# LarsELund/Bayesian-Neural-Nets

Measured on NVIDIA B200. Metric: train_samples_per_sec, higher is better.
Workload: dtype bf16

## Files before the change

### bayesian-neural-nets_b200/csrc/tc_gemm.cu

```cuda
#include <cuda.h>

#include <cstdlib>

#include "common.cuh"
#include "lrt_chain.cuh"
#include "tc_ptx.cuh"

namespace lbbnn {
namespace {

constexpr int BM = 128, BN = 128, BK = 64;
constexpr int UMMA_K = 16;
constexpr int kStages = 3;
constexpr int kTileBytes = BM * BK * 2;
constexpr int kStageBytes = 4 * kTileBytes;
constexpr int kEpiWarps = 8;
constexpr int kTcThreads = 64 + kEpiWarps * 32;
constexpr int kTmemCols = 512;
constexpr int EW = 16;
constexpr int kBiasBytes = 2 * 2 * BN * 4;
constexpr int kEpiScratchBytes = kEpiWarps * 4096;
static_assert(kEpiScratchBytes >= kBiasBytes, "scratch holds the bias terms too");
constexpr int kSmemBytes = kStages * kStageBytes + 1024  + 256  + kEpiScratchBytes;
constexpr int smem_for(int full, int mode) { return mode == LBBNN_TC_EPI_DW_ADAM ? full : full - kEpiScratchBytes + kBiasBytes; }

using namespace tc;

__host__ __device__ constexpr uint32_t make_idesc(int m, int n, int a_mn, int b_mn) {
  return (1u << 4) | (1u << 7) | (1u << 10) | ((uint32_t)(a_mn & 1) << 15) | ((uint32_t)(b_mn & 1) << 16) |
         ((uint32_t)(n >> 3) << 17) | ((uint32_t)(m >> 4) << 24);
}

__device__ __forceinline__ void umma_bf16(uint32_t tmem_d, uint64_t adesc, uint64_t bdesc, uint32_t idesc, uint32_t accumulate) {
  asm volatile(
      "{\n\t"
      ".reg .pred p;\n\t"
      "setp.ne.b32 p, %4, 0;\n\t"
      "tcgen05.mma.cta_group::1.kind::f16 [%0], %1, %2, %3, p;\n\t"
      "}" ::"r"(tmem_d),
      "l"(adesc), "l"(bdesc), "r"(idesc), "r"(accumulate)
      : "memory");
}

constexpr int kMnBoxBytes = 64 * 128;
__device__ __forceinline__ uint64_t umma_desc_mn_sw128(uint32_t smem_addr) {
  uint64_t d = 0;
  d |= (uint64_t)((smem_addr & 0x3FFFF) >> 4);
  d |= (uint64_t)(kMnBoxBytes >> 4) << 16;
  d |= (uint64_t)(1024 >> 4) << 32;
  d |= (uint64_t)1 << 46;
  d |= (uint64_t)2 << 61;
  return d;
}
__device__ __forceinline__ uint64_t umma_desc(uint32_t smem_addr, int mn) {
  return mn ? umma_desc_mn_sw128(smem_addr) : umma_desc_kmajor_sw128(smem_addr);
}

__device__ __forceinline__ uint32_t pack_bf16(float a, float b) {
  __nv_bfloat162 h = __floats2bfloat162_rn(a, b);
  return *reinterpret_cast<uint32_t*>(&h);
}

struct TcEpi {
  int mode;
  int flags;
  float *d1, *d2;
  const float *bias_mu, *bias_rho;
  Noise noise;
  __nv_bfloat16 *o_bf, *o2_bf, *oT_bf, *o2T_bf;
  float *o_f32, *dsf;
  const __nv_bfloat16* x_bf;
  const float* dsf_prev;
  __nv_bfloat16 *de, *ds, *deT, *dsT;
  float* colsum_part;
  float *p_mu, *p_rho, *p_lam;
  float *m_mu, *m_rho, *m_lam, *v_mu, *v_rho, *v_lam;
  const float* coef;
  lbbnn_priors pri;
  int var_mode;
  float klg, beta1, beta2, adam_eps;
  __nv_bfloat16 *next_M, *next_V;
  double* next_kl_part;
  int a_mn, b_mn;
  int l2_prefetch;
};

__device__ __forceinline__ float4 ld4(const float* p) { return *reinterpret_cast<const float4*>(p); }
__device__ __forceinline__ void st4(float* p, float a, float b, float c, float d) { *reinterpret_cast<float4*>(p) = make_float4(a, b, c, d); }

__device__ __forceinline__ void dw_adam_quad(const TcEpi& e, const chain::Consts& cc, const chain::KlC& kc, float& kl_acc, int64_t off,
                                             const float4 dM, const float4 dV) {
  const float4 mu4 = ld4(e.p_mu + off), rho4 = ld4(e.p_rho + off), lam4 = ld4(e.p_lam + off);
  const float4 mm4 = ld4(e.m_mu + off), mr4 = ld4(e.m_rho + off), ml4 = ld4(e.m_lam + off);
  const float4 vm4 = ld4(e.v_mu + off), vr4 = ld4(e.v_rho + off), vl4 = ld4(e.v_lam + off);
  float mu[4] = {mu4.x, mu4.y, mu4.z, mu4.w}, rho[4] = {rho4.x, rho4.y, rho4.z, rho4.w}, lam[4] = {lam4.x, lam4.y, lam4.z, lam4.w};
  float mm[4] = {mm4.x, mm4.y, mm4.z, mm4.w}, mr[4] = {mr4.x, mr4.y, mr4.z, mr4.w}, ml[4] = {ml4.x, ml4.y, ml4.z, ml4.w};
  float vm[4] = {vm4.x, vm4.y, vm4.z, vm4.w}, vr[4] = {vr4.x, vr4.y, vr4.z, vr4.w}, vl[4] = {vl4.x, vl4.y, vl4.z, vl4.w};
  const float d1[4] = {dM.x, dM.y, dM.z, dM.w}, d2[4] = {dV.x, dV.y, dV.z, dV.w};
#pragma unroll
  for (int t = 0; t < 4; ++t) {
    float gm, gr, gl;
    chain::grads(cc, mu[t], rho[t], lam[t], d1[t], d2[t], gm, gr, gl);
    chain::adam(cc, mu[t], mm[t], vm[t], gm);
    chain::adam(cc, rho[t], mr[t], vr[t], gr);
    chain::adam(cc, lam[t], ml[t], vl[t], gl);
  }
  st4(e.p_mu + off, mu[0], mu[1], mu[2], mu[3]); st4(e.p_rho + off, rho[0], rho[1], rho[2], rho[3]);
  st4(e.p_lam + off, lam[0], lam[1], lam[2], lam[3]);
  st4(e.m_mu + off, mm[0], mm[1], mm[2], mm[3]); st4(e.m_rho + off, mr[0], mr[1], mr[2], mr[3]);
  st4(e.m_lam + off, ml[0], ml[1], ml[2], ml[3]);
  st4(e.v_mu + off, vm[0], vm[1], vm[2], vm[3]); st4(e.v_rho + off, vr[0], vr[1], vr[2], vr[3]);
  st4(e.v_lam + off, vl[0], vl[1], vl[2], vl[3]);
  if (e.next_M) {
    float M[4], V[4];
#pragma unroll
    for (int t = 0; t < 4; ++t) {
      float k_;
      chain::next_moments(kc, cc.var_mode, mu[t], rho[t], lam[t], M[t], V[t], k_);
      kl_acc += k_;
    }
    uint2 pm, pv;
    pm.x = pack_bf16(M[0], M[1]); pm.y = pack_bf16(M[2], M[3]);
    pv.x = pack_bf16(V[0], V[1]); pv.y = pack_bf16(V[2], V[3]);
    *reinterpret_cast<uint2*>(e.next_M + off) = pm;
    *reinterpret_cast<uint2*>(e.next_V + off) = pv;
  }
}

__device__ __forceinline__ void dw_adam_tile(const TcEpi& e, const chain::Consts& cc, const chain::KlC& kc, float& kl_acc, int64_t M,
                                             int64_t N, int64_t row0, int64_t col0, uint32_t tbase, float* __restrict__ stg,
                                             int lane) {
#pragma unroll 1
  for (int c = 0; c < 64 / EW; ++c) {
    float v1[EW], v2[EW];
    tmem_ld16(tbase + c * EW, v1);
    tmem_ld16(tbase + 128 + c * EW, v2);
#pragma unroll
    for (int jj = 0; jj < 4; ++jj) {
      st4(stg + lane * 32 + ((jj ^ (lane & 7)) << 2), v1[4 * jj], v1[4 * jj + 1], v1[4 * jj + 2], v1[4 * jj + 3]);
      st4(stg + lane * 32 + (((4 + jj) ^ (lane & 7)) << 2), v2[4 * jj], v2[4 * jj + 1], v2[4 * jj + 2], v2[4 * jj + 3]);
    }
    __syncwarp();
    const int qd = lane & 3;
    const int64_t col = col0 + c * EW + qd * 4;
#pragma unroll
    for (int it = 0; it < 4; ++it) {
      const int rr = it * 8 + (lane >> 2);
      const float4 dM = ld4(stg + rr * 32 + ((qd ^ (rr & 7)) << 2));
      const float4 dV = ld4(stg + rr * 32 + (((4 + qd) ^ (rr & 7)) << 2));
      const int64_t row = row0 + rr;
      if (row < M && col < N) dw_adam_quad(e, cc, kc, kl_acc, row * N + col, dM, dV);
    }
    __syncwarp();
  }
}

__device__ __forceinline__ float warp_transpose_sum32(float (&vals)[32], int lane) {
#pragma unroll
  for (int s = 16; s >= 1; s >>= 1) {
    const bool up = lane & s;
#pragma unroll
    for (int i = 0; i < s; ++i) {
      const float send = up ? vals[i] : vals[i + s];
      const float keep = up ? vals[i + s] : vals[i];
      vals[i] = keep + __shfl_xor_sync(0xffffffffu, send, s);
    }
  }
  return vals[0];
}

template <int MODE>
__device__ __forceinline__ void epilogue_chunk(const TcEpi& e, const Noise& nz, const chain::Consts& cc, int64_t M, int64_t N,
                                               int64_t row, int64_t col0, const float* __restrict__ sbias, int cl,
                                               const float d1[EW], const float d2[EW]) {
  const bool row_ok = row < M;
  if (!row_ok && !(MODE == LBBNN_TC_EPI_DX && e.colsum_part)) return;
  const bool fullc = col0 + EW - 1 < N;
  if constexpr (MODE == LBBNN_TC_EPI_RAW) {
    float* p1 = e.d1 + row * N + col0;
    float* p2 = e.d2 + row * N + col0;
    if (fullc && (N % 4 == 0)) {
#pragma unroll
      for (int j = 0; j < EW; j += 4) {
        *reinterpret_cast<float4*>(p1 + j) = make_float4(d1[j], d1[j + 1], d1[j + 2], d1[j + 3]);
        *reinterpret_cast<float4*>(p2 + j) = make_float4(d2[j], d2[j + 1], d2[j + 2], d2[j + 3]);
      }
    } else {
#pragma unroll
      for (int j = 0; j < EW; ++j)
        if (col0 + j < N) { p1[j] = d1[j]; p2[j] = d2[j]; }
    }
    return;
  }
  float o[EW], o2[EW];
  if constexpr (MODE == LBBNN_TC_EPI_FWD) {
    float ep[EW];
    if (nz.ptr) {
#pragma unroll
      for (int j = 0; j < EW; ++j) ep[j] = (col0 + j < N) ? __ldg(nz.ptr + row * N + col0 + j) : 0.f;
    } else if (N % 4 == 0) {
#pragma unroll
      for (int j = 0; j < EW; j += 4) philox_normal4(nz.seed, nz.stream, ((uint64_t)row * (uint64_t)N + (uint64_t)(col0 + j)) >> 2, ep + j);
    } else {
#pragma unroll
      for (int j = 0; j < EW; ++j) ep[j] = philox_normal1(nz.seed, nz.stream, (uint64_t)row * (uint64_t)N + (uint64_t)(col0 + j));
    }
#pragma unroll
    for (int j = 0; j < EW; ++j) {
      const int64_t n = col0 + j;
      float v = 0.f, f = 0.f;
      if (n < N) {
        const float sd = sqrtf(fmaxf(d2[j], 0.f) + sbias[BN + cl + j]);
        v = d1[j] + sbias[cl + j] + sd * ep[j];
        f = ep[j] / (2.0f * sd);
        if (e.flags & LBBNN_FLAG_RELU) v = fmaxf(v, 0.f);
      }
      o[j] = v;
      o2[j] = f;
    }
    const bool v4 = fullc && (N % 4 == 0);
    if (e.o_f32 || e.dsf) {
      if (v4) {
#pragma unroll
        for (int j = 0; j < EW; j += 4) {
          if (e.o_f32) *reinterpret_cast<float4*>(e.o_f32 + row * N + col0 + j) = make_float4(o[j], o[j + 1], o[j + 2], o[j + 3]);
          if (e.dsf) *reinterpret_cast<float4*>(e.dsf + row * N + col0 + j) = make_float4(o2[j], o2[j + 1], o2[j + 2], o2[j + 3]);
        }
      } else {
#pragma unroll
        for (int j = 0; j < EW; ++j)
          if (col0 + j < N) {
            if (e.o_f32) e.o_f32[row * N + col0 + j] = o[j];
            if (e.dsf) e.dsf[row * N + col0 + j] = o2[j];
          }
      }
    }
    if (fullc && (N % 8 == 0)) {
#pragma unroll
      for (int j = 0; j < EW; j += 8) {
        uint4 a, b;
        a.x = pack_bf16(o[j], o[j + 1]); a.y = pack_bf16(o[j + 2], o[j + 3]); a.z = pack_bf16(o[j + 4], o[j + 5]); a.w = pack_bf16(o[j + 6], o[j + 7]);
        b.x = pack_bf16(o[j] * o[j], o[j + 1] * o[j + 1]); b.y = pack_bf16(o[j + 2] * o[j + 2], o[j + 3] * o[j + 3]);
        b.z = pack_bf16(o[j + 4] * o[j + 4], o[j + 5] * o[j + 5]); b.w = pack_bf16(o[j + 6] * o[j + 6], o[j + 7] * o[j + 7]);
        if (e.o_bf) *reinterpret_cast<uint4*>(e.o_bf + row * N + col0 + j) = a;
        if (e.o2_bf) *reinterpret_cast<uint4*>(e.o2_bf + row * N + col0 + j) = b;
      }
    } else {
#pragma unroll
      for (int j = 0; j < EW; ++j)
        if (col0 + j < N) {
          if (e.o_bf) e.o_bf[row * N + col0 + j] = __float2bfloat16_rn(o[j]);
          if (e.o2_bf) e.o2_bf[row * N + col0 + j] = __float2bfloat16_rn(o[j] * o[j]);
        }
    }
    if (e.oT_bf) {
#pragma unroll
      for (int j = 0; j < EW; ++j)
        if (col0 + j < N) {
          e.oT_bf[(col0 + j) * M + row] = __float2bfloat16_rn(o[j]);
          e.o2T_bf[(col0 + j) * M + row] = __float2bfloat16_rn(o[j] * o[j]);
        }
    }
    return;
  }
  if constexpr (MODE == LBBNN_TC_EPI_DX) {
  float xv[EW], fv[EW];
  if (!row_ok) {
#pragma unroll
    for (int j = 0; j < EW; ++j) { xv[j] = 0.f; fv[j] = 0.f; }
  } else if (fullc && (N % 8 == 0)) {
#pragma unroll
    for (int j = 0; j < EW; j += 8) {
      const uint4 u = *reinterpret_cast<const uint4*>(e.x_bf + row * N + col0 + j);
      const __nv_bfloat162* h = reinterpret_cast<const __nv_bfloat162*>(&u);
#pragma unroll
      for (int t = 0; t < 4; ++t) {
        const float2 f2 = __bfloat1622float2(h[t]);
        xv[j + 2 * t] = f2.x; xv[j + 2 * t + 1] = f2.y;
      }
    }
#pragma unroll
    for (int j = 0; j < EW; j += 4) {
      const float4 f4 = e.dsf_prev ? *reinterpret_cast<const float4*>(e.dsf_prev + row * N + col0 + j) : make_float4(0.f, 0.f, 0.f, 0.f);
      fv[j] = f4.x; fv[j + 1] = f4.y; fv[j + 2] = f4.z; fv[j + 3] = f4.w;
    }
  } else {
#pragma unroll
    for (int j = 0; j < EW; ++j) {
      const bool ok = col0 + j < N;
      xv[j] = ok ? __bfloat162float(e.x_bf[row * N + col0 + j]) : 0.f;
      fv[j] = (ok && e.dsf_prev) ? e.dsf_prev[row * N + col0 + j] : 0.f;
    }
  }
#pragma unroll
  for (int j = 0; j < EW; ++j) {
    float g = fmaf(2.0f * xv[j], d2[j], d1[j]);
    if ((e.flags & LBBNN_FLAG_MASK_DX) && !(xv[j] > 0.f)) g = 0.f;
    if (!row_ok || col0 + j >= N) g = 0.f;
    o[j] = g;
    o2[j] = g * fv[j];
  }
  if (e.colsum_part) {
    float vals[32];
#pragma unroll
    for (int j = 0; j < EW; ++j) { vals[j] = o[j]; vals[EW + j] = o2[j]; }
// ... 116 lines not shown
      constexpr uint64_t kbs = BMN ? (uint64_t)(2048 >> 4) : (uint64_t)((UMMA_K * 2) >> 4);
      for (int t = blockIdx.x; t < num_tiles; t += gridDim.x, ++it) {
        const int as = it & 1;
        mbar_wait(&tempty_bar[as], ((it >> 1) & 1) ^ 1);
        tc_fence_after();
        const uint32_t d1 = tmem_base + as * 256, d2 = d1 + 128;
        for (int kb = 0; kb < num_kb; ++kb) {
          mbar_wait(&full_bar[stage], phase);
          tc_fence_after();
          const uint32_t sa = smem_u32(smem + stage * kStageBytes);
          const uint64_t a1 = umma_desc(sa + 0 * kTileBytes, AMN), a2 = umma_desc(sa + 1 * kTileBytes, AMN);
          const uint64_t b1 = umma_desc(sa + 2 * kTileBytes, BMN), b2 = umma_desc(sa + 3 * kTileBytes, BMN);
#pragma unroll
          for (int k = 0; k < BK / UMMA_K; ++k) {
            const uint32_t acc = (kb | k) ? 1u : 0u;
            umma_bf16(d1, a1 + k * ka, b1 + k * kbs, idesc, acc);
            umma_bf16(d2, a2 + k * ka, b2 + k * kbs, idesc, acc);
          }
          umma_commit(&empty_bar[stage]);
          if (++stage == kStages) { stage = 0; phase ^= 1; }
        }
        umma_commit(&tfull_bar[as]);
      }
    }
  } else {
    Noise nz = epi.noise;
    nz.resolve();
    chain::Consts cc = {};
    chain::KlC kc = {};
    float kl_acc = 0.f;
    if constexpr (MODE == LBBNN_TC_EPI_DW_ADAM) {
      cc = chain::make_consts(epi.pri, epi.var_mode, epi.klg, epi.beta1, epi.beta2, epi.adam_eps, epi.coef);
      kc = chain::make_klc(epi.pri);
    }
    const int q = warp & 3, half = (warp - 2) >> 2;
    const int et = threadIdx.x - 64;
    int it = 0;
    for (int t = blockIdx.x; t < num_tiles; t += gridDim.x, ++it) {
      const int as = it & 1;
      int mb, nb;
      tile_coords(t, num_m, num_n, mb, nb);
      const int m0 = mb * BM, n0 = nb * BN;
      float* sbias = sbias_all + as * 2 * BN;
      if constexpr (MODE == LBBNN_TC_EPI_FWD) {
        const int c = et & (BN - 1);
        const int64_t n = n0 + c;
        float v = 0.f;
        if (n < N) {
          if (et < BN) v = __ldg(epi.bias_mu + n);
          else { const float sb = sigma_of(__ldg(epi.bias_rho + n)); v = sb * sb; }
        }
        sbias[(et < BN ? 0 : BN) + c] = v;
        asm volatile("bar.sync 1, %0;" ::"n"(kEpiWarps * 32) : "memory");
      }
      mbar_wait(&tfull_bar[as], (it >> 1) & 1);
      tc_fence_after();
      const int64_t row = m0 + q * 32 + lane;
      const uint32_t tbase = tmem_base + ((uint32_t)(q * 32) << 16) + as * 256 + half * 64;
      if constexpr (MODE == LBBNN_TC_EPI_DW_ADAM) {
        dw_adam_tile(epi, cc, kc, kl_acc, M, N, m0 + q * 32, n0 + half * 64, tbase, sbias_all + (warp - 2) * 1024, lane);
      } else {
#pragma unroll 1
        for (int c = 0; c < 64 / EW; ++c) {
          float v1[EW], v2[EW];
          tmem_ld16(tbase + c * EW, v1);
          tmem_ld16(tbase + 128 + c * EW, v2);
          const int cl = half * 64 + c * EW;
          epilogue_chunk<MODE>(epi, nz, cc, M, N, row, n0 + cl, sbias, cl, v1, v2);
        }
      }
      tc_fence_before();
      __syncwarp();
      if (lane == 0) mbar_arrive(&tempty_bar[as]);
    }
    if constexpr (MODE == LBBNN_TC_EPI_DW_ADAM) {
      if (epi.next_kl_part) {
        const float w = warp_sum(kl_acc);
        if (lane == 0) epi.next_kl_part[(int64_t)blockIdx.x * kEpiWarps + (warp - 2)] = (double)w;
      }
    }
  }
  tc_fence_before();
  __syncthreads();
  if (warp == 1) {
    tc_fence_after();
    tmem_dealloc(tmem_base, kTmemCols);
  }
}

constexpr int kStages2 = 4;
constexpr int kBHalfBytes = (BN / 2) * BK * 2;
constexpr int kStageBytes2 = 2 * kTileBytes + 2 * kBHalfBytes;
constexpr int kSmemBytes2 = kStages2 * kStageBytes2 + 1024 + 256 + kEpiScratchBytes;
static_assert(kSmemBytes <= 232448 && kSmemBytes2 <= 232448, "over the 227 KB shared-memory limit");
constexpr int kGroupM2 = kGroupM / 2;
constexpr int kL2Prefetch = 0;

__device__ __forceinline__ void umma_bf16_pair(uint32_t tmem_d, uint64_t adesc, uint64_t bdesc, uint32_t idesc, uint32_t accumulate) {
  asm volatile(
      "{\n\t"
      ".reg .pred p;\n\t"
      "setp.ne.b32 p, %4, 0;\n\t"
      "tcgen05.mma.cta_group::2.kind::f16 [%0], %1, %2, %3, p;\n\t"
      "}" ::"r"(tmem_d),
      "l"(adesc), "l"(bdesc), "r"(idesc), "r"(accumulate)
      : "memory");
}

__device__ __forceinline__ void tile_coords2(int t, int num_m2, int num_n, int group, int& mb2, int& nb) {
  const int per_group = group * num_n;
  const int g = t / per_group, r = t - g * per_group;
  const int m_first = g * group;
  const int gm = min(group, num_m2 - m_first);
  nb = r / gm;
  mb2 = m_first + (r - nb * gm);
}

template <int MODE, int AMN, int BMN>
__global__ void __cluster_dims__(2, 1, 1) __launch_bounds__(kTcThreads, 1)
tc_dual_gemm_bf16_pair(const __grid_constant__ CUtensorMap tmA1, const __grid_constant__ CUtensorMap tmA2,
                       const __grid_constant__ CUtensorMap tmB1, const __grid_constant__ CUtensorMap tmB2, const TcEpi epi,
                       int M, int N, int K, int group) {
  extern __shared__ uint8_t smem_raw[];
  uint8_t* smem = reinterpret_cast<uint8_t*>((reinterpret_cast<uintptr_t>(smem_raw) + 1023) & ~uintptr_t(1023));
  uint64_t* bars = reinterpret_cast<uint64_t*>(smem + kStages2 * kStageBytes2);
  uint64_t* full_bar = bars;
  uint64_t* empty_bar = bars + kStages2;
  uint64_t* tfull_bar = bars + 2 * kStages2;
  uint64_t* tempty_bar = bars + 2 * kStages2 + 2;
  uint32_t* tmem_holder = reinterpret_cast<uint32_t*>(bars + 2 * kStages2 + 4);
  float* sbias_all = reinterpret_cast<float*>(smem + kStages2 * kStageBytes2 + 256);

  const int warp = threadIdx.x >> 5, lane = threadIdx.x & 31;
  const uint32_t rank = cluster_ctarank();
  const int num_m2 = (M + 2 * BM - 1) / (2 * BM), num_n = (N + BN - 1) / BN;
  const int num_tiles = num_m2 * num_n, num_kb = (K + BK - 1) / BK;
  const int cluster_id = blockIdx.x >> 1, num_clusters = gridDim.x >> 1;

  if (warp == 0 && lane == 0) {
    tma_prefetch_desc(&tmA1); tma_prefetch_desc(&tmA2); tma_prefetch_desc(&tmB1); tma_prefetch_desc(&tmB2);
    for (int s = 0; s < kStages2; ++s) { mbar_init(&full_bar[s], 2); mbar_init(&empty_bar[s], 1); }
    for (int s = 0; s < 2; ++s) { mbar_init(&tfull_bar[s], 1); mbar_init(&tempty_bar[s], 2 * kEpiWarps); }
    fence_barrier_init();
  }
  __syncwarp();
  if (warp == 1) tmem_alloc_pair(tmem_holder, kTmemCols);
  tc_fence_before();
  cluster_sync_all();
  tc_fence_after();
  const uint32_t tmem_base = *tmem_holder;

  if (warp == 0) {
    if (lane == 0) {
      int stage = 0; uint32_t phase = 0;
      for (int t = cluster_id; t < num_tiles; t += num_clusters) {
        int mb2, nb;
        tile_coords2(t, num_m2, num_n, group, mb2, nb);
        const int m0 = mb2 * 2 * BM + (int)rank * BM, n0h = nb * BN + (int)rank * (BN / 2);
        for (int kb = 0; kb < num_kb; ++kb) {
          if (epi.l2_prefetch > 0) {
            int pk = kb + epi.l2_prefetch, pm0 = m0, pn0 = n0h;
            bool ok = true;
            if (pk >= num_kb) {
              pk -= num_kb;
              const int tn = t + num_clusters;
              ok = tn < num_tiles && pk < num_kb;
              if (ok) {
                int pmb2, pnb;
                tile_coords2(tn, num_m2, num_n, group, pmb2, pnb);
                pm0 = pmb2 * 2 * BM + (int)rank * BM; pn0 = pnb * BN + (int)rank * (BN / 2);
              }
            }
            if (ok) {
              if constexpr (!AMN) { tma_prefetch_l2_2d(&tmA1, pk * BK, pm0); tma_prefetch_l2_2d(&tmA2, pk * BK, pm0); }
              else {
#pragma unroll
                for (int h = 0; h < 2; ++h) { tma_prefetch_l2_2d(&tmA1, pm0 + 64 * h, pk * BK); tma_prefetch_l2_2d(&tmA2, pm0 + 64 * h, pk * BK); }
              }
              if constexpr (!BMN) { tma_prefetch_l2_2d(&tmB1, pk * BK, pn0); tma_prefetch_l2_2d(&tmB2, pk * BK, pn0); }
              else { tma_prefetch_l2_2d(&tmB1, pn0, pk * BK); tma_prefetch_l2_2d(&tmB2, pn0, pk * BK); }
            }
          }
          mbar_wait(&empty_bar[stage], phase ^ 1);
          uint8_t* sa = smem + stage * kStageBytes2;
          const uint32_t lead_full = mapa_u32(&full_bar[stage], 0);
          mbar_expect_tx_cluster(lead_full, kStageBytes2);
          if constexpr (!AMN) {
            tma_load_2d_pair(sa, &tmA1, lead_full, kb * BK, m0);
            tma_load_2d_pair(sa + kTileBytes, &tmA2, lead_full, kb * BK, m0);
          } else {
#pragma unroll
            for (int h = 0; h < 2; ++h) {
              tma_load_2d_pair(sa + h * kMnBoxBytes, &tmA1, lead_full, m0 + 64 * h, kb * BK);
              tma_load_2d_pair(sa + kTileBytes + h * kMnBoxBytes, &tmA2, lead_full, m0 + 64 * h, kb * BK);
            }
          }
          if constexpr (!BMN) {
            tma_load_2d_pair(sa + 2 * kTileBytes, &tmB1, lead_full, kb * BK, n0h);
            tma_load_2d_pair(sa + 2 * kTileBytes + kBHalfBytes, &tmB2, lead_full, kb * BK, n0h);
          } else {
            tma_load_2d_pair(sa + 2 * kTileBytes, &tmB1, lead_full, n0h, kb * BK);
            tma_load_2d_pair(sa + 2 * kTileBytes + kBHalfBytes, &tmB2, lead_full, n0h, kb * BK);
          }
          if (++stage == kStages2) { stage = 0; phase ^= 1; }
        }
      }
    }
  } else if (warp == 1) {
    if (lane == 0 && rank == 0) {
      int stage = 0; uint32_t phase = 0; int it = 0;
      constexpr uint32_t idesc = make_idesc(2 * BM, BN, AMN, BMN);
      constexpr uint64_t ka = AMN ? (uint64_t)(2048 >> 4) : (uint64_t)((UMMA_K * 2) >> 4);
      constexpr uint64_t kbs = BMN ? (uint64_t)(2048 >> 4) : (uint64_t)((UMMA_K * 2) >> 4);
      for (int t = cluster_id; t < num_tiles; t += num_clusters, ++it) {
        const int as = it & 1;
        mbar_wait(&tempty_bar[as], ((it >> 1) & 1) ^ 1);
        tc_fence_after();
        const uint32_t d1 = tmem_base + as * 256, d2 = d1 + 128;
        for (int kb = 0; kb < num_kb; ++kb) {
          mbar_wait(&full_bar[stage], phase);
          tc_fence_after();
          const uint32_t sa = smem_u32(smem + stage * kStageBytes2);
          const uint64_t a1 = umma_desc(sa, AMN), a2 = umma_desc(sa + kTileBytes, AMN);
          const uint64_t b1 = umma_desc(sa + 2 * kTileBytes, BMN);
          const uint64_t b2 = umma_desc(sa + 2 * kTileBytes + kBHalfBytes, BMN);
#pragma unroll
          for (int k = 0; k < BK / UMMA_K; ++k) {
            const uint32_t acc = (kb | k) ? 1u : 0u;
            umma_bf16_pair(d1, a1 + k * ka, b1 + k * kbs, idesc, acc);
            umma_bf16_pair(d2, a2 + k * ka, b2 + k * kbs, idesc, acc);
          }
          umma_commit_pair(&empty_bar[stage], 3);
          if (++stage == kStages2) { stage = 0; phase ^= 1; }
        }
        umma_commit_pair(&tfull_bar[as], 3);
      }
    }
  } else {
    Noise nz = epi.noise;
    nz.resolve();
    chain::Consts cc = {};
    chain::KlC kc = {};
    float kl_acc = 0.f;
    if constexpr (MODE == LBBNN_TC_EPI_DW_ADAM) {
      cc = chain::make_consts(epi.pri, epi.var_mode, epi.klg, epi.beta1, epi.beta2, epi.adam_eps, epi.coef);
      kc = chain::make_klc(epi.pri);
    }
    const int q = warp & 3, half = (warp - 2) >> 2;
    const int et = threadIdx.x - 64;
    int it = 0;
    for (int t = cluster_id; t < num_tiles; t += num_clusters, ++it) {
      const int as = it & 1;
      int mb2, nb;
      tile_coords2(t, num_m2, num_n, group, mb2, nb);
      const int m0 = mb2 * 2 * BM + (int)rank * BM, n0 = nb * BN;
      float* sbias = sbias_all + as * 2 * BN;
      if constexpr (MODE == LBBNN_TC_EPI_FWD) {
        const int c = et & (BN - 1);
        const int64_t n = n0 + c;
        float v = 0.f;
        if (n < N) {
          if (et < BN) v = __ldg(epi.bias_mu + n);
          else { const float sb = sigma_of(__ldg(epi.bias_rho + n)); v = sb * sb; }
        }
        sbias[(et < BN ? 0 : BN) + c] = v;
        asm volatile("bar.sync 1, %0;" ::"n"(kEpiWarps * 32) : "memory");
      }
      mbar_wait(&tfull_bar[as], (it >> 1) & 1);
      tc_fence_after();
      const int64_t row = m0 + q * 32 + lane;
      const uint32_t tbase = tmem_base + ((uint32_t)(q * 32) << 16) + as * 256 + half * 64;
      if constexpr (MODE == LBBNN_TC_EPI_DW_ADAM) {
        dw_adam_tile(epi, cc, kc, kl_acc, M, N, m0 + q * 32, n0 + half * 64, tbase, sbias_all + (warp - 2) * 1024, lane);
      } else {
#pragma unroll 1
        for (int c = 0; c < 64 / EW; ++c) {
          float v1[EW], v2[EW];
          tmem_ld16(tbase + c * EW, v1);
          tmem_ld16(tbase + 128 + c * EW, v2);
          const int cl = half * 64 + c * EW;
          epilogue_chunk<MODE>(epi, nz, cc, M, N, row, n0 + cl, sbias, cl, v1, v2);
        }
      }
      tc_fence_before();
      __syncwarp();
      if (lane == 0) mbar_arrive_cluster(mapa_u32(&tempty_bar[as], 0));
    }
    if constexpr (MODE == LBBNN_TC_EPI_DW_ADAM) {
      if (epi.next_kl_part) {
        const float w = warp_sum(kl_acc);
        if (lane == 0) epi.next_kl_part[(int64_t)blockIdx.x * kEpiWarps + (warp - 2)] = (double)w;
      }
    }
  }
  __syncwarp();
  tc_fence_before();
  cluster_sync_all();
  if (warp == 1) {
    tc_fence_after();
    tmem_dealloc_pair(tmem_base, kTmemCols);
  }
}

typedef CUresult (*EncodeTiledFn)(CUtensorMap*, CUtensorMapDataType, cuuint32_t, void*, const cuuint64_t*, const cuuint64_t*,
                                  const cuuint32_t*, const cuuint32_t*, CUtensorMapInterleave, CUtensorMapSwizzle,
                                  CUtensorMapL2promotion, CUtensorMapFloatOOBfill);

EncodeTiledFn get_encode() {
  static EncodeTiledFn fn = nullptr;
  if (fn) return fn;
  void* p = nullptr;
  cudaDriverEntryPointQueryResult qres;
  if (cudaGetDriverEntryPoint("cuTensorMapEncodeTiled", &p, cudaEnableDefault, &qres) != cudaSuccess ||
      qres != cudaDriverEntryPointSuccess)
    return nullptr;
  fn = (EncodeTiledFn)p;
  return fn;
}

int make_map(CUtensorMap* map, const void* ptr, int64_t rows, int64_t K, int box_rows = BM) {
  EncodeTiledFn enc = get_encode();
  LBBNN_REQUIRE(enc != nullptr, "cuTensorMapEncodeTiled not available from the driver");
  LBBNN_REQUIRE((reinterpret_cast<uintptr_t>(ptr) & 15) == 0 && (K * 2) % 16 == 0,
                "TMA operand must be 16B aligned with a 16B-multiple row pitch (K %% 8 == 0), K=%lld", (long long)K);
  cuuint64_t dims[2] = {(cuuint64_t)K, (cuuint64_t)rows};
  cuuint64_t strides[1] = {(cuuint64_t)K * 2};
  cuuint32_t box[2] = {(cuuint32_t)BK, (cuuint32_t)box_rows};
  cuuint32_t estr[2] = {1, 1};
  CUresult r = enc(map, CU_TENSOR_MAP_DATA_TYPE_BFLOAT16, 2, const_cast<void*>(ptr), dims, strides, box, estr,
                   CU_TENSOR_MAP_INTERLEAVE_NONE, CU_TENSOR_MAP_SWIZZLE_128B, CU_TENSOR_MAP_L2_PROMOTION_L2_256B,
                   CU_TENSOR_MAP_FLOAT_OOB_FILL_NONE);
  LBBNN_REQUIRE(r == CUDA_SUCCESS, "cuTensorMapEncodeTiled failed (%d) rows=%lld K=%lld", (int)r, (long long)rows, (long long)K);
  return LBBNN_OK;
}

int make_map_mn(CUtensorMap* map, const void* ptr, int64_t rows, int64_t K) {
  EncodeTiledFn enc = get_encode();
  LBBNN_REQUIRE(enc != nullptr, "cuTensorMapEncodeTiled not available from the driver");
  LBBNN_REQUIRE((reinterpret_cast<uintptr_t>(ptr) & 15) == 0 && (rows * 2) % 16 == 0,
                "MN-major TMA operand must be 16B aligned with a 16B-multiple row pitch (rows %% 8 == 0), rows=%lld", (long long)rows);
  cuuint64_t dims[2] = {(cuuint64_t)rows, (cuuint64_t)K};
  cuuint64_t strides[1] = {(cuuint64_t)rows * 2};
  cuuint32_t box[2] = {64u, (cuuint32_t)BK};
  cuuint32_t estr[2] = {1, 1};
  CUresult r = enc(map, CU_TENSOR_MAP_DATA_TYPE_BFLOAT16, 2, const_cast<void*>(ptr), dims, strides, box, estr,
                   CU_TENSOR_MAP_INTERLEAVE_NONE, CU_TENSOR_MAP_SWIZZLE_128B, CU_TENSOR_MAP_L2_PROMOTION_L2_256B,
                   CU_TENSOR_MAP_FLOAT_OOB_FILL_NONE);
  LBBNN_REQUIRE(r == CUDA_SUCCESS, "cuTensorMapEncodeTiled (MN-major) failed (%d) rows=%lld K=%lld", (int)r, (long long)rows, (long long)K);
  return LBBNN_OK;
}

int launch_tc(const void* A1, const void* A2, const void* B1, const void* B2, int64_t M, int64_t N, int64_t K, const TcEpi& epi_in,
              cudaStream_t st) {
  LBBNN_REQUIRE(A1 && A2 && B1 && B2 && M > 0 && N > 0 && K > 0, "bad GEMM operands");
  TcEpi epi = epi_in;
  {
    const char* pf = getenv("LBBNN_TC_L2_PREFETCH");
    epi.l2_prefetch = pf ? atoi(pf) : kL2Prefetch;
  }
  LBBNN_REQUIRE(M < (1LL << 31) && N < (1LL << 31) && K < (1LL << 31), "GEMM dims must fit int32");
  CUtensorMap mA1, mA2, mB1, mB2;
  if (epi.a_mn) {
    if (int rc = make_map_mn(&mA1, A1, M, K)) return rc;
    if (int rc = make_map_mn(&mA2, A2, M, K)) return rc;
  } else {
    if (int rc = make_map(&mA1, A1, M, K)) return rc;
    if (int rc = make_map(&mA2, A2, M, K)) return rc;
  }
  const char* pe = getenv("LBBNN_TC_PAIR");
  const int pair_mode = pe ? atoi(pe) : 1;
  const int64_t tiles2 = ceil_div(M, 2 * BM) * ceil_div(N, BN);
  if (pair_mode && M > BM && (pair_mode == 2 || tiles2 >= sm_count() / 2)) {
    if (epi.b_mn) {
      if (int rc = make_map_mn(&mB1, B1, N, K)) return rc;
      if (int rc = make_map_mn(&mB2, B2, N, K)) return rc;
    } else {
      if (int rc = make_map(&mB1, B1, N, K, BN / 2)) return rc;
      if (int rc = make_map(&mB2, B2, N, K, BN / 2)) return rc;
    }
    const int clusters = (int)(tiles2 < sm_count() / 2 ? tiles2 : sm_count() / 2);
    const char* ge = getenv("LBBNN_TC_GROUP");
    const int group = ge && atoi(ge) > 0 ? atoi(ge) : kGroupM2;
    const int key = epi.mode * 4 + epi.a_mn * 2 + epi.b_mn;
    switch (key) {
#define LBBNN_PAIR_CASE(MODE_, A_, B_)                                                                                                \
  case (MODE_) * 4 + (A_) * 2 + (B_): {                                                                                              \
    static bool attr_set_ = false;                                                                                                   \
    if (!attr_set_) {                                                                                                                \
      LBBNN_CUDA(cudaFuncSetAttribute(tc_dual_gemm_bf16_pair<MODE_, A_, B_>, cudaFuncAttributeMaxDynamicSharedMemorySize,           \
                                      smem_for(kSmemBytes2, MODE_)));                                                               \
      attr_set_ = true;                                                                                                              \
    }                                                                                                                                \
    tc_dual_gemm_bf16_pair<MODE_, A_, B_><<<2 * clusters, kTcThreads, smem_for(kSmemBytes2, MODE_), st>>>(mA1, mA2, mB1, mB2, epi, \
                                                                                                           (int)M, (int)N, (int)K, \
                                                                                                           group);                 \
    break;                                                                                                                           \
  }
      LBBNN_PAIR_CASE(LBBNN_TC_EPI_RAW, 0, 0)
      LBBNN_PAIR_CASE(LBBNN_TC_EPI_RAW, 0, 1)
      LBBNN_PAIR_CASE(LBBNN_TC_EPI_RAW, 1, 0)
      LBBNN_PAIR_CASE(LBBNN_TC_EPI_RAW, 1, 1)
      LBBNN_PAIR_CASE(LBBNN_TC_EPI_FWD, 0, 0)
      LBBNN_PAIR_CASE(LBBNN_TC_EPI_DX, 0, 0)
      LBBNN_PAIR_CASE(LBBNN_TC_EPI_DX, 0, 1)
      LBBNN_PAIR_CASE(LBBNN_TC_EPI_DW_ADAM, 1, 1)
#undef LBBNN_PAIR_CASE
      default: LBBNN_REQUIRE(false, "no kernel for epilogue mode %d with operand majors (%d, %d)", epi.mode, epi.a_mn, epi.b_mn);
    }
    return check_launch("tc_dual_gemm_bf16_pair");
  }
  if (epi.b_mn) {
    if (int rc = make_map_mn(&mB1, B1, N, K)) return rc;
    if (int rc = make_map_mn(&mB2, B2, N, K)) return rc;
  } else {
    if (int rc = make_map(&mB1, B1, N, K)) return rc;
    if (int rc = make_map(&mB2, B2, N, K)) return rc;
  }
  const int64_t tiles = ceil_div(M, BM) * ceil_div(N, BN);
  const int grid = (int)(tiles < sm_count() ? tiles : sm_count());
  const int key = epi.mode * 4 + epi.a_mn * 2 + epi.b_mn;
  switch (key) {
#define LBBNN_ONE_CASE(MODE_, A_, B_)                                                                                          \
  case (MODE_) * 4 + (A_) * 2 + (B_): {                                                                                       \
    static bool attr_set_ = false;                                                                                             \
    if (!attr_set_) {                                                                                                          \
      LBBNN_CUDA(cudaFuncSetAttribute(tc_dual_gemm_bf16<MODE_, A_, B_>, cudaFuncAttributeMaxDynamicSharedMemorySize,          \
                                      smem_for(kSmemBytes, MODE_)));                                                          \
      attr_set_ = true;                                                                                                        \
    }                                                                                                                          \
    tc_dual_gemm_bf16<MODE_, A_, B_><<<grid, kTcThreads, smem_for(kSmemBytes, MODE_), st>>>(mA1, mA2, mB1, mB2, epi, (int)M,   \
                                                                                             (int)N, (int)K);                   \
    break;                                                                                                                     \
  }
    LBBNN_ONE_CASE(LBBNN_TC_EPI_RAW, 0, 0)
    LBBNN_ONE_CASE(LBBNN_TC_EPI_RAW, 0, 1)
    LBBNN_ONE_CASE(LBBNN_TC_EPI_RAW, 1, 0)
    LBBNN_ONE_CASE(LBBNN_TC_EPI_RAW, 1, 1)
    LBBNN_ONE_CASE(LBBNN_TC_EPI_FWD, 0, 0)
    LBBNN_ONE_CASE(LBBNN_TC_EPI_DX, 0, 0)
    LBBNN_ONE_CASE(LBBNN_TC_EPI_DX, 0, 1)
    LBBNN_ONE_CASE(LBBNN_TC_EPI_DW_ADAM, 1, 1)
#undef LBBNN_ONE_CASE
    default: LBBNN_REQUIRE(false, "no kernel for epilogue mode %d with operand majors (%d, %d)", epi.mode, epi.a_mn, epi.b_mn);
  }
  return check_launch("tc_dual_gemm_bf16");
}

}
}

using namespace lbbnn;

extern "C" int lbbnn_tc_dual_gemm_raw(const void* A1, const void* A2, const void* B1, const void* B2, int64_t M, int64_t N,
                                      int64_t K, float* D1, float* D2, lbbnn_stream s) {
  LBBNN_REQUIRE(D1 && D2, "NULL output");
  TcEpi e = {};
  e.mode = LBBNN_TC_EPI_RAW;
  e.d1 = D1; e.d2 = D2;
  return launch_tc(A1, A2, B1, B2, M, N, K, e, (cudaStream_t)s);
}

extern "C" int lbbnn_tc_lrt_fwd(const void* x_bf, const void* x2_bf, const void* M_bf, const void* V_bf, int64_t batch,
                                int64_t in_features, int64_t out_features, const float* bias_mu, const float* bias_rho,
                                const lbbnn_noise* nz, int flags, void* act_bf, void* act2_bf, void* actT_bf, void* act2T_bf,
                                float* ds_factor, float* act_f32, lbbnn_stream s) {
  LBBNN_REQUIRE(bias_mu && bias_rho, "NULL bias");
  LBBNN_REQUIRE((actT_bf == nullptr) == (act2T_bf == nullptr), "transposed outputs come in pairs");
  TcEpi e = {};
  e.mode = LBBNN_TC_EPI_FWD; e.flags = flags;
  e.bias_mu = bias_mu; e.bias_rho = bias_rho; e.noise = make_noise(nz);
  e.o_bf = (__nv_bfloat16*)act_bf; e.o2_bf = (__nv_bfloat16*)act2_bf; e.oT_bf = (__nv_bfloat16*)actT_bf;
  e.o2T_bf = (__nv_bfloat16*)act2T_bf; e.dsf = ds_factor; e.o_f32 = act_f32;
  return launch_tc(x_bf, x2_bf, M_bf, V_bf, batch, out_features, in_features, e, (cudaStream_t)s);
}

extern "C" int lbbnn_tc_lrt_bwd_input(const void* dE_bf, const void* dS_bf, const void* MT_bf, const void* VT_bf, int64_t batch,
                                      int64_t in_features, int64_t out_features, const void* x_bf, const float* ds_factor_prev,
                                      int flags, void* dE_prev_bf, void* dS_prev_bf, void* dE_prevT_bf, void* dS_prevT_bf,
                                      lbbnn_stream s) {
  LBBNN_REQUIRE(x_bf && dE_prev_bf && dS_prev_bf, "NULL argument");
  LBBNN_REQUIRE((dE_prevT_bf == nullptr) == (dS_prevT_bf == nullptr), "transposed outputs come in pairs");
  TcEpi e = {};
  e.mode = LBBNN_TC_EPI_DX; e.flags = flags;
  e.x_bf = (const __nv_bfloat16*)x_bf; e.dsf_prev = ds_factor_prev;
  e.de = (__nv_bfloat16*)dE_prev_bf; e.ds = (__nv_bfloat16*)dS_prev_bf; e.deT = (__nv_bfloat16*)dE_prevT_bf;
  e.dsT = (__nv_bfloat16*)dS_prevT_bf;
  return launch_tc(dE_bf, dS_bf, MT_bf, VT_bf, batch, in_features, out_features, e, (cudaStream_t)s);
}

namespace lbbnn {
namespace {
__global__ void __launch_bounds__(256) colsum_part_reduce(const float* __restrict__ part, int n_part, int64_t cols2,
                                                          float* __restrict__ out) {
  const int64_t c = (int64_t)blockIdx.x * blockDim.x + threadIdx.x;
  if (c >= cols2) return;
  float s = 0.f;
  for (int r = 0; r < n_part; ++r) s += part[(int64_t)r * cols2 + c];
  out[c] = s;
}
}
}

extern "C" int lbbnn_tc_dual_gemm_raw_ex(const void* A1, const void* A2, const void* B1, const void* B2, int64_t M, int64_t N,
                                         int64_t K, int a_mn, int b_mn, float* D1, float* D2, lbbnn_stream s) {
  LBBNN_REQUIRE(D1 && D2, "NULL output");
  TcEpi e = {};
  e.mode = LBBNN_TC_EPI_RAW;
  e.d1 = D1; e.d2 = D2;
  e.a_mn = a_mn ? 1 : 0; e.b_mn = b_mn ? 1 : 0;
  return launch_tc(A1, A2, B1, B2, M, N, K, e, (cudaStream_t)s);
}

extern "C" size_t lbbnn_tc_colsum_part_floats(int64_t batch, int64_t in_features) {
  return (size_t)(ceil_div(batch, 32) * 2 * in_features);
}

extern "C" int lbbnn_tc_colsum_reduce(const float* part, int64_t batch, int64_t in_features, float* colsum, lbbnn_stream s) {
  LBBNN_REQUIRE(part && colsum && batch > 0 && in_features > 0, "bad argument");
  const int64_t cols2 = 2 * in_features;
  colsum_part_reduce<<<(unsigned)ceil_div(cols2, 256), 256, 0, (cudaStream_t)s>>>(part, (int)ceil_div(batch, 32), cols2, colsum);
  return check_launch("colsum_part_reduce");
}

extern "C" int lbbnn_tc_lrt_bwd_input_mn(const void* dE_bf, const void* dS_bf, const void* M_bf, const void* V_bf, int64_t batch,
                                         int64_t in_features, int64_t out_features, const void* x_bf, const float* ds_factor_prev,
                                         int flags, void* dE_prev_bf, void* dS_prev_bf, float* colsum_part, lbbnn_stream s) {
  LBBNN_REQUIRE(x_bf && dE_prev_bf && dS_prev_bf, "NULL argument");
  TcEpi e = {};
  e.mode = LBBNN_TC_EPI_DX; e.flags = flags;
  e.x_bf = (const __nv_bfloat16*)x_bf; e.dsf_prev = ds_factor_prev;
  e.de = (__nv_bfloat16*)dE_prev_bf; e.ds = (__nv_bfloat16*)dS_prev_bf;
  e.colsum_part = colsum_part;
  e.a_mn = 0; e.b_mn = 1;
  return launch_tc(dE_bf, dS_bf, M_bf, V_bf, batch, in_features, out_features, e, (cudaStream_t)s);
}

extern "C" size_t lbbnn_tc_lrt_dw_adam_kl_parts(void) { return (size_t)sm_count() * kEpiWarps; }

extern "C" int lbbnn_tc_lrt_dw_adam_next(const void* dE_bf, const void* dS_bf, const void* x_bf, const void* x2_bf,
                                         const lbbnn_layer* L, int64_t batch, const lbbnn_priors* pri, int var_mode,
                                         float kl_grad, const lbbnn_adam_layer_state* adam, void* next_M_bf, void* next_V_bf,
                                         double* next_kl_part, lbbnn_stream s);

extern "C" int lbbnn_tc_lrt_dw_adam(const void* dE_bf, const void* dS_bf, const void* x_bf, const void* x2_bf,
                                    const lbbnn_layer* L, int64_t batch, const lbbnn_priors* pri, int var_mode,
                                    float kl_grad, const lbbnn_adam_layer_state* adam, lbbnn_stream s) {
  return lbbnn_tc_lrt_dw_adam_next(dE_bf, dS_bf, x_bf, x2_bf, L, batch, pri, var_mode, kl_grad, adam, nullptr, nullptr, nullptr, s);
}

extern "C" int lbbnn_tc_lrt_dw_adam_next(const void* dE_bf, const void* dS_bf, const void* x_bf, const void* x2_bf,
                                         const lbbnn_layer* L, int64_t batch, const lbbnn_priors* pri, int var_mode,
                                         float kl_grad, const lbbnn_adam_layer_state* adam, void* next_M_bf, void* next_V_bf,
                                         double* next_kl_part, lbbnn_stream s) {
  LBBNN_REQUIRE((next_M_bf == nullptr) == (next_V_bf == nullptr), "next_M / next_V come in pairs");
  LBBNN_REQUIRE(next_kl_part == nullptr || next_M_bf != nullptr, "next_kl_part needs next_M / next_V");
  LBBNN_REQUIRE(L && pri && adam && adam->coef, "NULL argument");
  LBBNN_REQUIRE(L->weight_mu && L->weight_rho && L->lambdal && L->in_features > 0 && L->out_features > 0, "bad layer");
  LBBNN_REQUIRE(L->z == nullptr && L->z_kl == nullptr, "the fused update is for LRT layers (no multiplicative z)");
  LBBNN_REQUIRE(L->in_features % 8 == 0 && L->out_features % 8 == 0, "fused dW update needs in/out features divisible by 8");
  for (int i = 0; i < 3; ++i) LBBNN_REQUIRE(adam->exp_avg[i] && adam->exp_avg_sq[i], "NULL Adam state %d", i);
  TcEpi e = {};
  e.mode = LBBNN_TC_EPI_DW_ADAM;
  e.p_mu = const_cast<float*>(L->weight_mu); e.p_rho = const_cast<float*>(L->weight_rho); e.p_lam = const_cast<float*>(L->lambdal);
  e.m_mu = adam->exp_avg[0]; e.m_rho = adam->exp_avg[1]; e.m_lam = adam->exp_avg[2];
  e.v_mu = adam->exp_avg_sq[0]; e.v_rho = adam->exp_avg_sq[1]; e.v_lam = adam->exp_avg_sq[2];
  const float* ptrs[9] = {e.p_mu, e.p_rho, e.p_lam, e.m_mu, e.m_rho, e.m_lam, e.v_mu, e.v_rho, e.v_lam};
  for (int i = 0; i < 9; ++i) LBBNN_REQUIRE((reinterpret_cast<uintptr_t>(ptrs[i]) & 15) == 0, "parameters / Adam state must be 16B aligned");
  e.coef = adam->coef; e.pri = *pri; e.var_mode = var_mode; e.klg = kl_grad;
  e.beta1 = adam->beta1; e.beta2 = adam->beta2; e.adam_eps = adam->eps;
  e.next_M = (__nv_bfloat16*)next_M_bf; e.next_V = (__nv_bfloat16*)next_V_bf; e.next_kl_part = next_kl_part;
  if (next_kl_part)
    LBBNN_CUDA(cudaMemsetAsync(next_kl_part, 0, lbbnn_tc_lrt_dw_adam_kl_parts() * sizeof(double), (cudaStream_t)s));
  e.a_mn = 1; e.b_mn = 1;
  return launch_tc(dE_bf, dS_bf, x_bf, x2_bf, L->out_features, L->in_features, batch, e, (cudaStream_t)s);
}
```

Before: 2.507 million.

## Add staged 256x256 pair GEMM kernel stashing pass results in L2

Adds a new 2-CTA cluster kernel for forward and dX modes. It computes the two GEMMs (mu and variance passes) back to back, each into its own 256-column TMEM accumulator over a 256x256 cluster tile, so each operand tile covers more output per load. Because TMEM cannot hold both full results for the epilogue, the first pass's results are spilled to a per-SM global stash with L2 evict_last hints and read back with evict_first before the fused epilogue. This trades less operand traffic and deeper 6-stage pipelining against extra stash traffic through L2, a one-time host-synchronising allocation, and an assumption of one CTA per SM that is only enforced by the shared-memory size.

```diff
diff --git a/bayesian-neural-nets_b200/csrc/tc_gemm.cu b/bayesian-neural-nets_b200/csrc/tc_gemm.cu
--- a/bayesian-neural-nets_b200/csrc/tc_gemm.cu
+++ b/bayesian-neural-nets_b200/csrc/tc_gemm.cu
@@ -1,6 +1,7 @@
 #include <cuda.h>
 
 #include <cstdlib>
+#include <mutex>
 
 #include "common.cuh"
 #include "lrt_chain.cuh"
@@ -723,6 +724,194 @@
   }
 }
 
+constexpr int kStagesS = 6;
+constexpr int kStageBytesS = 2 * kTileBytes;
+constexpr int kBiasBytesS = 2 * 2 * 2 * BN * 4;
+constexpr int kSmemBytesS = kStagesS * kStageBytesS + 1024 + 256 + kBiasBytesS;
+static_assert(kSmemBytesS <= 232448, "over the 227 KB shared-memory limit");
+static_assert(kSmemBytesS > 232448 / 2, "the stash slot per %smid needs at most one CTA per SM");
+constexpr int kStashFloats = 2 * BM * 2 * BN;
+
+__device__ __forceinline__ uint32_t smid_u32() {
+  uint32_t r;
+  asm volatile("mov.u32 %0, %%smid;" : "=r"(r));
+  return r;
+}
+__device__ __forceinline__ void st_stash(float* p, float a, float b, float c, float d, uint64_t pol) {
+  asm volatile("st.global.L1::no_allocate.L2::cache_hint.v4.f32 [%0], {%1, %2, %3, %4}, %5;" ::"l"(p), "f"(a), "f"(b), "f"(c),
+               "f"(d), "l"(pol)
+               : "memory");
+}
+__device__ __forceinline__ float4 ld_stash(const float* p, uint64_t pol) {
+  float4 v;
+  asm volatile("ld.global.L1::no_allocate.L2::cache_hint.v4.f32 {%0, %1, %2, %3}, [%4], %5;"
+               : "=f"(v.x), "=f"(v.y), "=f"(v.z), "=f"(v.w)
+               : "l"(p), "l"(pol));
+  return v;
+}
+
+template <int MODE, int AMN, int BMN>
+__global__ void __cluster_dims__(2, 1, 1) __launch_bounds__(kTcThreads, 1)
+tc_gemm_bf16_pair_staged(const __grid_constant__ CUtensorMap tmA1, const __grid_constant__ CUtensorMap tmA2,
+                         const __grid_constant__ CUtensorMap tmB1, const __grid_constant__ CUtensorMap tmB2, const TcEpi epi,
+                         int M, int N, int K, int group, float* __restrict__ stash) {
+  extern __shared__ uint8_t smem_raw[];
+  uint8_t* smem = reinterpret_cast<uint8_t*>((reinterpret_cast<uintptr_t>(smem_raw) + 1023) & ~uintptr_t(1023));
+  uint64_t* bars = reinterpret_cast<uint64_t*>(smem + kStagesS * kStageBytesS);
+  uint64_t* full_bar = bars;
+  uint64_t* empty_bar = bars + kStagesS;
+  uint64_t* tfull_bar = bars + 2 * kStagesS;
+  uint64_t* tempty_bar = bars + 2 * kStagesS + 2;
+  uint32_t* tmem_holder = reinterpret_cast<uint32_t*>(bars + 2 * kStagesS + 4);
+  float* sbias_all = reinterpret_cast<float*>(smem + kStagesS * kStageBytesS + 256);
+
+  const int warp = threadIdx.x >> 5, lane = threadIdx.x & 31;
+  const uint32_t rank = cluster_ctarank();
+  const int num_m2 = (M + 2 * BM - 1) / (2 * BM), num_n2 = (N + 2 * BN - 1) / (2 * BN);
+  const int num_tiles = num_m2 * num_n2, num_kb = (K + BK - 1) / BK;
+  const int cluster_id = blockIdx.x >> 1, num_clusters = gridDim.x >> 1;
+
+  if (warp == 0 && lane == 0) {
+    tma_prefetch_desc(&tmA1); tma_prefetch_desc(&tmA2); tma_prefetch_desc(&tmB1); tma_prefetch_desc(&tmB2);
+    for (int s = 0; s < kStagesS; ++s) { mbar_init(&full_bar[s], 2); mbar_init(&empty_bar[s], 1); }
+    for (int s = 0; s < 2; ++s) { mbar_init(&tfull_bar[s], 1); mbar_init(&tempty_bar[s], 2 * kEpiWarps); }
+    fence_barrier_init();
+  }
+  __syncwarp();
+  if (warp == 1) tmem_alloc_pair(tmem_holder, kTmemCols);
+  tc_fence_before();
+  cluster_sync_all();
+  tc_fence_after();
+  const uint32_t tmem_base = *tmem_holder;
+
+  if (warp == 0) {
+    if (lane == 0) {
+      int stage = 0; uint32_t phase = 0;
+      for (int t = cluster_id; t < num_tiles; t += num_clusters) {
+        int mb2, nb2;
+        tile_coords2(t, num_m2, num_n2, group, mb2, nb2);
+        const int m0 = mb2 * 2 * BM + (int)rank * BM, n0h = nb2 * 2 * BN + (int)rank * BN;
+        for (int pass = 0; pass < 2; ++pass) {
+          const CUtensorMap* ta = pass ? &tmA2 : &tmA1;
+          const CUtensorMap* tb = pass ? &tmB2 : &tmB1;
+          for (int kb = 0; kb < num_kb; ++kb) {
+            mbar_wait(&empty_bar[stage], phase ^ 1);
+            uint8_t* sa = smem + stage * kStageBytesS;
+            const uint32_t lead_full = mapa_u32(&full_bar[stage], 0);
+            mbar_expect_tx_cluster(lead_full, kStageBytesS);
+            if constexpr (!AMN) {
+              tma_load_2d_pair(sa, ta, lead_full, kb * BK, m0);
+            } else {
+#pragma unroll
+              for (int h = 0; h < 2; ++h) tma_load_2d_pair(sa + h * kMnBoxBytes, ta, lead_full, m0 + 64 * h, kb * BK);
+            }
+            if constexpr (!BMN) {
+              tma_load_2d_pair(sa + kTileBytes, tb, lead_full, kb * BK, n0h);
+            } else {
+#pragma unroll
+              for (int h = 0; h < 2; ++h) tma_load_2d_pair(sa + kTileBytes + h * kMnBoxBytes, tb, lead_full, n0h + 64 * h, kb * BK);
+            }
+            if (++stage == kStagesS) { stage = 0; phase ^= 1; }
+          }
+        }
+      }
+    }
+  } else if (warp == 1) {
+    if (lane == 0 && rank == 0) {
+      int stage = 0; uint32_t phase = 0; int it = 0;
+      constexpr uint32_t idesc = make_idesc(2 * BM, 2 * BN, AMN, BMN);
+      constexpr uint64_t ka = AMN ? (uint64_t)(2048 >> 4) : (uint64_t)((UMMA_K * 2) >> 4);
+      constexpr uint64_t kbs = BMN ? (uint64_t)(2048 >> 4) : (uint64_t)((UMMA_K * 2) >> 4);
+      for (int t = cluster_id; t < num_tiles; t += num_clusters, ++it) {
+        for (int pass = 0; pass < 2; ++pass) {
+          mbar_wait(&tempty_bar[pass], (it & 1) ^ 1);
+          tc_fence_after();
+          const uint32_t d = tmem_base + pass * 256;
+          for (int kb = 0; kb < num_kb; ++kb) {
+            mbar_wait(&full_bar[stage], phase);
+            tc_fence_after();
+            const uint32_t sa = smem_u32(smem + stage * kStageBytesS);
+            const uint64_t a = umma_desc(sa, AMN), b = umma_desc(sa + kTileBytes, BMN);
+#pragma unroll
+            for (int k = 0; k < BK / UMMA_K; ++k) umma_bf16_pair(d, a + k * ka, b + k * kbs, idesc, (kb | k) ? 1u : 0u);
+            umma_commit_pair(&empty_bar[stage], 3);
+            if (++stage == kStagesS) { stage = 0; phase ^= 1; }
+          }
+          umma_commit_pair(&tfull_bar[pass], 3);
+        }
+      }
+    }
+  } else {
+    Noise nz = epi.noise;
+    nz.resolve();
+    const chain::Consts cc = {};
+    const int q = warp & 3, half = (warp - 2) >> 2;
+    const int et = threadIdx.x - 64;
+    float* slot = stash + (size_t)smid_u32() * kStashFloats + (size_t)(warp - 2) * (2 * 8 * 4 * 32 * 4) + lane * 4;
+    constexpr int kProd = 8 * 4 * 32 * 4;
+    uint64_t pol_keep, pol_drop;
+    asm volatile("createpolicy.fractional.L2::evict_last.b64 %0, 1.0;" : "=l"(pol_keep));
+    asm volatile("createpolicy.fractional.L2::evict_first.b64 %0, 1.0;" : "=l"(pol_drop));
+    int it = 0;
+    for (int t = cluster_id; t < num_tiles; t += num_clusters, ++it) {
+      int mb2, nb2;
+      tile_coords2(t, num_m2, num_n2, group, mb2, nb2);
+      const int m0 = mb2 * 2 * BM + (int)rank * BM, n0 = nb2 * 2 * BN;
+      float* sbias = sbias_all + (it & 1) * 4 * BN;
+      if constexpr (MODE == LBBNN_TC_EPI_FWD) {
+        const int64_t n = n0 + et;
+        float bm = 0.f, sb2 = 0.f;
+        if (n < N) {
+          bm = __ldg(epi.bias_mu + n);
+          const float sb = sigma_of(__ldg(epi.bias_rho + n));
+          sb2 = sb * sb;
+        }
+        float* sb_h = sbias + (et / BN) * 2 * BN + (et % BN);
+        sb_h[0] = bm;
+        sb_h[BN] = sb2;
+        asm volatile("bar.sync 1, %0;" ::"n"(kEpiWarps * 32) : "memory");
+      }
+      const int64_t row = m0 + q * 32 + lane;
+      const uint32_t tbase = tmem_base + ((uint32_t)(q * 32) << 16) + half * BN;
+#pragma unroll 1
+      for (int pass = 0; pass < 2; ++pass) {
+        mbar_wait(&tfull_bar[pass], it & 1);
+        tc_fence_after();
+#pragma unroll 1
+        for (int c = 0; c < BN / EW; ++c) {
+          float v[EW];
+          tmem_ld16(tbase + pass * 256 + c * EW, v);
+#pragma unroll
+          for (int j = 0; j < EW / 4; ++j)
+            st_stash(slot + pass * kProd + (c * 4 + j) * 128, v[4 * j], v[4 * j + 1], v[4 * j + 2], v[4 * j + 3], pol_keep);
+        }
+        tc_fence_before();
+        __syncwarp();
+        if (lane == 0) mbar_arrive_cluster(mapa_u32(&tempty_bar[pass], 0));
+      }
+#pragma unroll 1
+      for (int c = 0; c < BN / EW; ++c) {
+        float v1[EW], v2[EW];
+#pragma unroll
+        for (int j = 0; j < EW / 4; ++j) {
+          const float4 s1 = ld_stash(slot + (c * 4 + j) * 128, pol_drop);
+          const float4 s2 = ld_stash(slot + kProd + (c * 4 + j) * 128, pol_drop);
+          v1[4 * j] = s1.x; v1[4 * j + 1] = s1.y; v1[4 * j + 2] = s1.z; v1[4 * j + 3] = s1.w;
+          v2[4 * j] = s2.x; v2[4 * j + 1] = s2.y; v2[4 * j + 2] = s2.z; v2[4 * j + 3] = s2.w;
+        }
+        epilogue_chunk<MODE>(epi, nz, cc, M, N, row, n0 + half * BN + c * EW, sbias + half * 2 * BN, c * EW, v1, v2);
+      }
+    }
+  }
+  __syncwarp();
+  tc_fence_before();
+  cluster_sync_all();
+  if (warp == 1) {
+    tc_fence_after();
+    tmem_dealloc_pair(tmem_base, kTmemCols);
+  }
+}
+
 typedef CUresult (*EncodeTiledFn)(CUtensorMap*, CUtensorMapDataType, cuuint32_t, void*, const cuuint64_t*, const cuuint64_t*,
                                   const cuuint32_t*, const cuuint32_t*, CUtensorMapInterleave, CUtensorMapSwizzle,
                                   CUtensorMapL2promotion, CUtensorMapFloatOOBfill);
@@ -771,6 +960,39 @@
   return LBBNN_OK;
 }
 
+__global__ void read_nsmid(int* out) {
+  uint32_t r;
+  asm volatile("mov.u32 %0, %%nsmid;" : "=r"(r));
+  *out = (int)r;
+}
+
+int staged_stash(cudaStream_t st, float** out) {
+  constexpr int kMaxDevices = 64;
+  static std::mutex mu;
+  static float* bufs[kMaxDevices] = {};
+  *out = nullptr;
+  int dev = 0;
+  LBBNN_CUDA(cudaGetDevice(&dev));
+  LBBNN_REQUIRE(dev < kMaxDevices, "device ordinal %d", dev);
+  std::lock_guard<std::mutex> lock(mu);
+  if (!bufs[dev]) {
+    cudaStreamCaptureStatus cs = cudaStreamCaptureStatusNone;
+    LBBNN_CUDA(cudaStreamIsCapturing(st, &cs));
+    if (cs != cudaStreamCaptureStatusNone) return LBBNN_OK;
+    int* d_n = nullptr;
+    int n = 0;
+    LBBNN_CUDA(cudaMalloc(&d_n, sizeof(int)));
+    read_nsmid<<<1, 1, 0, st>>>(d_n);
+    LBBNN_CUDA(cudaMemcpyAsync(&n, d_n, sizeof(int), cudaMemcpyDeviceToHost, st));
+    LBBNN_CUDA(cudaStreamSynchronize(st));
+    LBBNN_CUDA(cudaFree(d_n));
+    LBBNN_REQUIRE(n > 0, "%%nsmid = %d", n);
+    LBBNN_CUDA(cudaMalloc(&bufs[dev], (size_t)n * kStashFloats * sizeof(float)));
+  }
+  *out = bufs[dev];
+  return LBBNN_OK;
+}
+
 int launch_tc(const void* A1, const void* A2, const void* B1, const void* B2, int64_t M, int64_t N, int64_t K, const TcEpi& epi_in,
               cudaStream_t st) {
   LBBNN_REQUIRE(A1 && A2 && B1 && B2 && M > 0 && N > 0 && K > 0, "bad GEMM operands");
@@ -790,6 +1012,45 @@
   }
   const char* pe = getenv("LBBNN_TC_PAIR");
   const int pair_mode = pe ? atoi(pe) : 1;
+  const char* ge = getenv("LBBNN_TC_GROUP");
+  const int group = ge && atoi(ge) > 0 ? atoi(ge) : kGroupM2;
+  const char* se = getenv("LBBNN_TC_STAGED");
+  const int staged_mode = se ? atoi(se) : 1;
+  const bool staged_epi = !epi.a_mn && (epi.mode == LBBNN_TC_EPI_DX || (epi.mode == LBBNN_TC_EPI_FWD && !epi.b_mn));
+  const int64_t tiles_s = ceil_div(M, 2 * BM) * ceil_div(N, 2 * BN);
+  if (pair_mode && staged_mode && staged_epi && M > BM && (staged_mode == 2 || (M > 2 * BM && tiles_s >= sm_count() / 2))) {
+    float* stash = nullptr;
+    if (int rc = staged_stash(st, &stash)) return rc;
+    if (stash) {
+      if (epi.b_mn) {
+        if (int rc = make_map_mn(&mB1, B1, N, K)) return rc;
+        if (int rc = make_map_mn(&mB2, B2, N, K)) return rc;
+      } else {
+        if (int rc = make_map(&mB1, B1, N, K)) return rc;
+        if (int rc = make_map(&mB2, B2, N, K)) return rc;
+      }
+      const int clusters = (int)(tiles_s < sm_count() / 2 ? tiles_s : sm_count() / 2);
+      switch (epi.mode * 4 + epi.b_mn) {
+#define LBBNN_STAGED_CASE(MODE_, B_)                                                                                          \
+  case (MODE_) * 4 + (B_): {                                                                                                  \
+    static bool attr_set_ = false;                                                                                            \
+    if (!attr_set_) {                                                                                                         \
+      LBBNN_CUDA(cudaFuncSetAttribute(tc_gemm_bf16_pair_staged<MODE_, 0, B_>, cudaFuncAttributeMaxDynamicSharedMemorySize,   \
+                                      kSmemBytesS));                                                                          \
+      attr_set_ = true;                                                                                                       \
+    }                                                                                                                         \
+    tc_gemm_bf16_pair_staged<MODE_, 0, B_><<<2 * clusters, kTcThreads, kSmemBytesS, st>>>(mA1, mA2, mB1, mB2, epi, (int)M,    \
+                                                                                          (int)N, (int)K, group, stash);      \
+    break;                                                                                                                    \
+  }
+        LBBNN_STAGED_CASE(LBBNN_TC_EPI_FWD, 0)
+        LBBNN_STAGED_CASE(LBBNN_TC_EPI_DX, 0)
+        LBBNN_STAGED_CASE(LBBNN_TC_EPI_DX, 1)
+#undef LBBNN_STAGED_CASE
+      }
+      return check_launch("tc_gemm_bf16_pair_staged");
+    }
+  }
   const int64_t tiles2 = ceil_div(M, 2 * BM) * ceil_div(N, BN);
   if (pair_mode && M > BM && (pair_mode == 2 || tiles2 >= sm_count() / 2)) {
     if (epi.b_mn) {
@@ -800,8 +1061,6 @@
       if (int rc = make_map(&mB2, B2, N, K, BN / 2)) return rc;
     }
     const int clusters = (int)(tiles2 < sm_count() / 2 ? tiles2 : sm_count() / 2);
-    const char* ge = getenv("LBBNN_TC_GROUP");
-    const int group = ge && atoi(ge) > 0 ? atoi(ge) : kGroupM2;
     const int key = epi.mode * 4 + epi.a_mn * 2 + epi.b_mn;
     switch (key) {
 #define LBBNN_PAIR_CASE(MODE_, A_, B_)                                                                                                \
```

Result: no change. 2.512 million (median of 6 runs) (+0.2%).
